# kensho-technologies/pyctcdecode

Measured on AMD Instinct MI355X. Metric: logit-frames/sec (whole node) at beam=100, V=1024, 4-gram LM, higher is better.
Workload: dtype f64

## Files before the change

### pyctcdecode_amd/csrc/frame_prune_hip.hip

```cpp
#include <hip/hip_runtime.h>
#include <hip/hip_fp16.h>
#include <algorithm>
#include <type_traits>
#include <vector>
#include <math.h>
#include <stdlib.h>

#include "backend.h"
#include "set_order.h"
#include "np_f32.h"
#include "set_order_small.h"
#include "np_sum.h"
#include "wave_ops_hip.h"
#include "hip_try.h"
#include "prune_route.h"

namespace ctc {
namespace be {

template <typename T>
__device__ __forceinline__ double ld(const T* p, size_t i) {
  return (double)p[i];
}
struct half_bits { uint16_t u; };
// ... 490 lines not shown
__global__ __launch_bounds__(PRUNE_WAVES * 64) void frame_prune_listed(PruneArgs a, uint32_t cap) {
  extern __shared__ __attribute__((aligned(16))) char smem[];
  const int lane = threadIdx.x & 63;
  const int wave = threadIdx.x >> 6;
  const PruneLds w = prune_lds(smem, wave, (uint32_t)a.max_surv, cap);
  const uint32_t count = a.overflow[3];
  for (uint32_t k = blockIdx.x * PRUNE_WAVES + wave; k < count; k += gridDim.x * PRUNE_WAVES) {
    prune_row_generic<T>(a, a.row_base + (int64_t)a.slow_rows[k], w, lane);
    __builtin_amdgcn_wave_barrier();
    __threadfence_block();
  }
}

__device__ __forceinline__ double exp_nonpos(double d) {
  d = fmax(d, -750.0);
  const double kf = rint(d * 1.44269504088896338700e+00);
  double r = fma(kf, -6.93147180369123816490e-01, d);
  r = fma(kf, -1.90821492927058770002e-10, r);
  double p = 1.6059043836821613e-10;
  p = fma(p, r, 2.08767569878680990e-09);
  p = fma(p, r, 2.50521083854417188e-08);
  p = fma(p, r, 2.75573192239858907e-07);
  p = fma(p, r, 2.75573192239858907e-06);
  p = fma(p, r, 2.48015873015873016e-05);
  p = fma(p, r, 1.98412698412698413e-04);
  p = fma(p, r, 1.38888888888888889e-03);
  p = fma(p, r, 8.33333333333333333e-03);
  p = fma(p, r, 4.16666666666666667e-02);
  p = fma(p, r, 1.66666666666666667e-01);
  p = fma(p, r, 5.00000000000000000e-01);
  p = fma(p, r, 1.0);
  p = fma(p, r, 1.0);
  return ldexp(p, (int)kf);
}

__device__ __forceinline__ double exp_nonpos9(double d) {
  d = fmax(d, -750.0);
  const double kf = rint(d * 1.44269504088896338700e+00);
  double r = fma(kf, -6.93147180369123816490e-01, d);
  r = fma(kf, -1.90821492927058770002e-10, r);
  double p = 2.75573192239858907e-06;
  p = fma(p, r, 2.48015873015873016e-05);
  p = fma(p, r, 1.98412698412698413e-04);
  p = fma(p, r, 1.38888888888888889e-03);
  p = fma(p, r, 8.33333333333333333e-03);
  p = fma(p, r, 4.16666666666666667e-02);
  p = fma(p, r, 1.66666666666666667e-01);
  p = fma(p, r, 5.00000000000000000e-01);
  p = fma(p, r, 1.0);
  p = fma(p, r, 1.0);
  return ldexp(p, (int)kf);
}

typedef float f32x2 __attribute__((ext_vector_type(2)));
__device__ __forceinline__ f32x2 exp_nonpos_f32x2(f32x2 d) {
  d = __builtin_elementwise_max(d, (f32x2)(-80.0f));
  const f32x2 n = __builtin_elementwise_roundeven(d * (f32x2)(1.44269504088896340736f));
  f32x2 r = __builtin_elementwise_fma(n, (f32x2)(-0.693145751953125f), d);
  r = __builtin_elementwise_fma(n, (f32x2)(-1.42860682030941723212e-6f), r);
  f32x2 p = (f32x2)(2.48015873015873016e-05f);
  p = __builtin_elementwise_fma(p, r, (f32x2)(1.98412698412698413e-04f));
  p = __builtin_elementwise_fma(p, r, (f32x2)(1.38888888888888889e-03f));
  p = __builtin_elementwise_fma(p, r, (f32x2)(8.33333333333333333e-03f));
  p = __builtin_elementwise_fma(p, r, (f32x2)(4.16666666666666667e-02f));
  p = __builtin_elementwise_fma(p, r, (f32x2)(1.66666666666666667e-01f));
  p = __builtin_elementwise_fma(p, r, (f32x2)(0.5f));
  p = __builtin_elementwise_fma(p, r, (f32x2)(1.0f));
  p = __builtin_elementwise_fma(p, r, (f32x2)(1.0f));
  f32x2 out;
  out.x = ldexpf(p.x, (int)n.x);
  out.y = ldexpf(p.y, (int)n.y);
  return out;
}

__device__ __forceinline__ double log_ge1(double s) {
  const double y0 = (double)__logf((float)s);
  const double r = fma(s, exp_nonpos(-y0), -1.0);
  return y0 + (r - 0.5 * r * r);
}

template <int NC, bool PK>
__device__ __forceinline__ void prune_row_f32x4(const PruneArgs& a, int64_t row, const PruneLds& w, int lane) {
  const int V = a.n_labels;
  const int u = find_utt(a.utt_row0, a.n_utts, row);
  const bool is_prob = a.pass == 1;
  if (is_prob && a.utt_is_prob[u] != 1u) return;
  const float4* x4 = (const float4*)((const float*)a.utt_logits[u] + (size_t)(row - a.utt_row0[u]) * V);
  const int n4 = V >> 2;
  float4 r[NC];
#pragma unroll
  for (int k = 0; k < NC; ++k) {
    const int i4 = k * 64 + lane;
    r[k] = i4 < n4 ? x4[i4] : make_float4(-INFINITY, -INFINITY, -INFINITY, -INFINITY);
  }
  double mx = 0.0, lse = 0.0;
  const uint32_t ms = (uint32_t)a.max_surv;
  const unsigned long long lt = (1ull << lane) - 1ull;
  if (!is_prob) {
    float mf = -INFINITY;
    float rsf = 0.f;
#pragma unroll
    for (int k = 0; k < NC; ++k) {
      if (k * 64 + lane < n4) {
        mf = fmaxf(fmaxf(mf, fmaxf(r[k].x, r[k].y)), fmaxf(r[k].z, r[k].w));
        rsf += (r[k].x + r[k].y) + (r[k].z + r[k].w);
      }
    }
    double m = wave_max((double)mf);
    double rs = wave_sum((double)rsf);
    if (lane == 0) a.row_sum[row] = rs;
    if (isfinite(m) && rs == rs) {
      const float mfw = (float)m;
      double sl = 0.0;
      float l32 = 0.f;
      const bool np32 = a.f32_np != 0;
      if (np32) l32 = np_log_f32(np_order_exp_sum<float>((const float*)x4, V, mfw, lane, w));
#pragma unroll
      for (int k = 0; k < NC; ++k) {
        if (!np32 && k * 64 + lane < n4) {
          if (PK) {
            const f32x2 e01 = exp_nonpos_f32x2((f32x2){r[k].x - mfw, r[k].y - mfw});
            const f32x2 e23 = exp_nonpos_f32x2((f32x2){r[k].z - mfw, r[k].w - mfw});
            sl += ((double)e01.x + (double)e01.y) + ((double)e23.x + (double)e23.y);
          } else {
            sl += (exp_nonpos9((double)r[k].x - m) + exp_nonpos9((double)r[k].y - m)) +
                  (exp_nonpos9((double)r[k].z - m) + exp_nonpos9((double)r[k].w - m));
          }
        }
      }
      if (!np32) {
        const double s = wave_sum(sl);
        lse = log_ge1(s);
      } else {
        lse = (double)l32;
      }
      int first = 0x7FFFFFFF;
#pragma unroll
      for (int k = NC - 1; k >= 0; --k) {
        const int v0 = (k * 64 + lane) * 4;
        if (k * 64 + lane < n4) {
          first = r[k].w == mfw ? v0 + 3 : first;
          first = r[k].z == mfw ? v0 + 2 : first;
          first = r[k].y == mfw ? v0 + 1 : first;
          first = r[k].x == mfw ? v0 : first;
        }
      }
      first = wave_min_i32(first);
      const double best = np32 ? to_logp_np32(mfw, false, mfw, l32) : to_logp((double)mfw, false, m, lse);
      const double xthr = m + lse + a.token_min_logp;
      const float pre = a.token_min_logp <= -34.538776394910684 ? -INFINITY
                                                                  : __double2float_rd(xthr - (np32 ? 3e-5 * (4.0 + fabs(xthr)) : 1e-6 * (1.0 + fabs(xthr))));
      uint32_t n = 0;
#pragma unroll
      for (int k = 0; k < NC; ++k) {
        const bool in = k * 64 + lane < n4;
        const bool cand = in && (r[k].x >= pre || r[k].y >= pre || r[k].z >= pre || r[k].w >= pre);
        if (__ballot(cand)) {
          const int v0 = (k * 64 + lane) * 4;
          double y0 = -INFINITY, y1 = -INFINITY, y2 = -INFINITY, y3 = -INFINITY;
          if (cand && np32) {
            y0 = to_logp_np32(r[k].x, false, mfw, l32);
            y1 = to_logp_np32(r[k].y, false, mfw, l32);
            y2 = to_logp_np32(r[k].z, false, mfw, l32);
            y3 = to_logp_np32(r[k].w, false, mfw, l32);
          } else if (cand) {
            y0 = to_logp((double)r[k].x, false, m, lse);
            y1 = to_logp((double)r[k].y, false, m, lse);
            y2 = to_logp((double)r[k].z, false, m, lse);
            y3 = to_logp((double)r[k].w, false, m, lse);
          }
          const bool k0 = cand && y0 >= a.token_min_logp, k1 = cand && y1 >= a.token_min_logp;
          const bool k2 = cand && y2 >= a.token_min_logp, k3 = cand && y3 >= a.token_min_logp;
          const unsigned long long b0 = __ballot(k0), b1 = __ballot(k1), b2 = __ballot(k2), b3 = __ballot(k3);
          uint32_t pos = n + (uint32_t)(__popcll(b0 & lt) + __popcll(b1 & lt) + __popcll(b2 & lt) + __popcll(b3 & lt));
          if (k0) { if (pos < ms) { w.asc_id[pos] = (uint16_t)v0; w.asc_lp[pos] = y0; } ++pos; }
          if (k1) { if (pos < ms) { w.asc_id[pos] = (uint16_t)(v0 + 1); w.asc_lp[pos] = y1; } ++pos; }
          if (k2) { if (pos < ms) { w.asc_id[pos] = (uint16_t)(v0 + 2); w.asc_lp[pos] = y2; } ++pos; }
          if (k3) { if (pos < ms) { w.asc_id[pos] = (uint16_t)(v0 + 3); w.asc_lp[pos] = y3; } ++pos; }
          n += (uint32_t)(__popcll(b0) + __popcll(b1) + __popcll(b2) + __popcll(b3));
        }
      }
      prune_finish(a, row, lane, w, n, best, first, true);
      return;
    }
    if (!isfinite(m)) m = 0.0;
    double s = 0.0;
#pragma unroll
    for (int k = 0; k < NC; ++k) {
      if (k * 64 + lane < n4)
        s += (exp((double)r[k].x - m) + exp((double)r[k].y - m)) + (exp((double)r[k].z - m) + exp((double)r[k].w - m));
    }
    s = wave_sum(s);
    mx = m;
    lse = log(s);
  }
  uint32_t n = 0;
  double best = -INFINITY;
  int best_id = 0x7FFFFFFF;
#pragma unroll
  for (int k = 0; k < NC; ++k) {
    const bool in = k * 64 + lane < n4;
    const int v0 = (k * 64 + lane) * 4;
    double y0 = -INFINITY, y1 = -INFINITY, y2 = -INFINITY, y3 = -INFINITY;
    if (in && is_prob && a.f32_np) {
      y0 = to_logp_np32(r[k].x, true, 0.f, 0.f);
      y1 = to_logp_np32(r[k].y, true, 0.f, 0.f);
      y2 = to_logp_np32(r[k].z, true, 0.f, 0.f);
      y3 = to_logp_np32(r[k].w, true, 0.f, 0.f);
    } else if (in) {
      y0 = to_logp((double)r[k].x, is_prob, mx, lse);
      y1 = to_logp((double)r[k].y, is_prob, mx, lse);
      y2 = to_logp((double)r[k].z, is_prob, mx, lse);
      y3 = to_logp((double)r[k].w, is_prob, mx, lse);
    }
    if (in) {
      argmax_take(y0, v0, best, best_id);
      argmax_take(y1, v0 + 1, best, best_id);
      argmax_take(y2, v0 + 2, best, best_id);
      argmax_take(y3, v0 + 3, best, best_id);
    }
    const bool k0 = in && y0 >= a.token_min_logp, k1 = in && y1 >= a.token_min_logp;
    const bool k2 = in && y2 >= a.token_min_logp, k3 = in && y3 >= a.token_min_logp;
    const unsigned long long any = __ballot(k0 || k1 || k2 || k3);
    if (any) {
      const unsigned long long b0 = __ballot(k0), b1 = __ballot(k1), b2 = __ballot(k2), b3 = __ballot(k3);
      uint32_t pos = n + (uint32_t)(__popcll(b0 & lt) + __popcll(b1 & lt) + __popcll(b2 & lt) + __popcll(b3 & lt));
      if (k0) { if (pos < ms) { w.asc_id[pos] = (uint16_t)v0; w.asc_lp[pos] = y0; } ++pos; }
      if (k1) { if (pos < ms) { w.asc_id[pos] = (uint16_t)(v0 + 1); w.asc_lp[pos] = y1; } ++pos; }
      if (k2) { if (pos < ms) { w.asc_id[pos] = (uint16_t)(v0 + 2); w.asc_lp[pos] = y2; } ++pos; }
      if (k3) { if (pos < ms) { w.asc_id[pos] = (uint16_t)(v0 + 3); w.asc_lp[pos] = y3; } ++pos; }
      n += (uint32_t)(__popcll(b0) + __popcll(b1) + __popcll(b2) + __popcll(b3));
    }
  }
  prune_finish(a, row, lane, w, n, best, best_id);
}
template <int NC, bool PK>
__global__ __launch_bounds__(PRUNE_WAVES * 64) void frame_prune_f32x4(PruneArgs a, uint32_t cap) {
  extern __shared__ __attribute__((aligned(16))) char smem[];
  const int lane = threadIdx.x & 63;
  const int wave = threadIdx.x >> 6;
  const int64_t row = a.row_base + (int64_t)blockIdx.x * PRUNE_WAVES + wave;
  if (row >= a.row_base + a.n_rows) return;
  prune_row_f32x4<NC, PK>(a, row, prune_lds(smem, wave, (uint32_t)a.max_surv, cap), lane);
}
template <int NC>
__global__ __launch_bounds__(PRUNE_WAVES * 64) void frame_prune_f32x4_listed(PruneArgs a, uint32_t cap) {
  extern __shared__ __attribute__((aligned(16))) char smem[];
  const int lane = threadIdx.x & 63;
  const int wave = threadIdx.x >> 6;
  const PruneLds w = prune_lds(smem, wave, (uint32_t)a.max_surv, cap);
  const uint32_t count = a.overflow[3];
  for (uint32_t k = blockIdx.x * PRUNE_WAVES + wave; k < count; k += gridDim.x * PRUNE_WAVES) {
    prune_row_f32x4<NC, true>(a, a.row_base + (int64_t)a.slow_rows[k], w, lane);
    __builtin_amdgcn_wave_barrier();
    __threadfence_block();
  }
}

constexpr int PF_ROWS = 64;
constexpr int PF_CAND = 16;
constexpr int PF_WAVES = 3;
constexpr int NP_IL = 2;
constexpr size_t PF_LDS_IDS = (size_t)PF_ROWS * PF_CAND * 2;
constexpr size_t PF_LDS_X = (size_t)PF_ROWS * PF_CAND * 4;
static_assert(PRUNE_FAST_MAX_LABELS - 1 <= (int)SMALL_SET_MAX_ID, "label ids must fit the small set tables");
constexpr size_t PF_LDS = PF_LDS_IDS + PF_LDS_X + (size_t)PF_ROWS * SMALL_SET_SLOTS * 2;

__device__ __forceinline__ f32x2 exp_nonpos_f32x2m(f32x2 d) {
  d.x = fmaxf(d.x, -80.0f);
  d.y = fmaxf(d.y, -80.0f);
  const f32x2 magic = (f32x2)(12582912.0f);
  const f32x2 t = __builtin_elementwise_fma(d, (f32x2)(1.44269504088896340736f), magic);
  const f32x2 n = t - magic;
  f32x2 r = __builtin_elementwise_fma(n, (f32x2)(-0.693145751953125f), d);
  r = __builtin_elementwise_fma(n, (f32x2)(-1.42860682030941723212e-6f), r);
  f32x2 p = (f32x2)(1.98412698412698413e-04f);
  p = __builtin_elementwise_fma(p, r, (f32x2)(1.38888888888888889e-03f));
  p = __builtin_elementwise_fma(p, r, (f32x2)(8.33333333333333333e-03f));
  p = __builtin_elementwise_fma(p, r, (f32x2)(4.16666666666666667e-02f));
  p = __builtin_elementwise_fma(p, r, (f32x2)(1.66666666666666667e-01f));
  p = __builtin_elementwise_fma(p, r, (f32x2)(0.5f));
  p = __builtin_elementwise_fma(p, r, (f32x2)(1.0f));
  p = __builtin_elementwise_fma(p, r, (f32x2)(1.0f));
  f32x2 out;
  out.x = __uint_as_float(__float_as_uint(p.x) + (__float_as_uint(t.x) << 23));
  out.y = __uint_as_float(__float_as_uint(p.y) + (__float_as_uint(t.y) << 23));
  return out;
}

template <int CTRL, int ROW_MASK>
__device__ __forceinline__ float dpp_f32(float ident, float v) {
  return __int_as_float(__builtin_amdgcn_update_dpp(__float_as_int(ident), __float_as_int(v), CTRL, ROW_MASK, 0xf, false));
}
__device__ __forceinline__ float min3_raw(float a, float b, float c) {
  float o;
  asm("v_min3_f32 %0, %1, %2, %3" : "=v"(o) : "v"(a), "v"(b), "v"(c));
  return o;
}
__device__ __forceinline__ float max3_raw(float a, float b, float c) {
  float o;
  asm("v_max3_f32 %0, %1, %2, %3" : "=v"(o) : "v"(a), "v"(b), "v"(c));
  return o;
}
#define CTC_MAX_DPP(V, CTRL) asm volatile("s_nop 1\n\tv_max_f32_dpp %0, %0, %0 " CTRL : "+v"(V))
__device__ __forceinline__ float wave_max_f32(float v) {
  CTC_MAX_DPP(v, "row_shr:1 row_mask:0xf bank_mask:0xf");
  CTC_MAX_DPP(v, "row_shr:2 row_mask:0xf bank_mask:0xf");
  CTC_MAX_DPP(v, "row_shr:4 row_mask:0xf bank_mask:0xf");
  CTC_MAX_DPP(v, "row_shr:8 row_mask:0xf bank_mask:0xf");
  CTC_MAX_DPP(v, "row_bcast:15 row_mask:0xa bank_mask:0xf");
  CTC_MAX_DPP(v, "row_bcast:31 row_mask:0xc bank_mask:0xf");
  asm volatile("s_nop 1" ::: "memory");
  return __int_as_float(__builtin_amdgcn_readlane(__float_as_int(v), 63));
}
__device__ __forceinline__ float wave_sum_f32(float v) {
  v += dpp_f32<0x111, 0xf>(0.f, v);
  v += dpp_f32<0x112, 0xf>(0.f, v);
  v += dpp_f32<0x114, 0xf>(0.f, v);
  v += dpp_f32<0x118, 0xf>(0.f, v);
  v += dpp_f32<0x142, 0xa>(0.f, v);
  v += dpp_f32<0x143, 0xc>(0.f, v);
  return __int_as_float(__builtin_amdgcn_readlane(__float_as_int(v), 63));
}
__device__ __forceinline__ uint32_t lanes_below(uint64_t mask) {
  return __builtin_amdgcn_mbcnt_hi((uint32_t)(mask >> 32), __builtin_amdgcn_mbcnt_lo((uint32_t)mask, 0u));
}

struct LaneTab {
  uint16_t* t;
  __device__ __forceinline__ uint16_t get(uint32_t k) const { return t[k * PF_ROWS]; }
  __device__ __forceinline__ void put(uint32_t k, uint16_t v) { t[k * PF_ROWS] = v; }
};

typedef float PfF4 __attribute__((ext_vector_type(4)));
typedef uint32_t PfU4 __attribute__((ext_vector_type(4)));
template <int DT>
struct PfRaw {
  typedef PfF4 type;
};
template <>
struct PfRaw<2> {
  typedef PfU4 type;
};
template <>
struct PfRaw<3> {
  typedef PfU4 type;
};
template <int DT>
__device__ __forceinline__ float pf_widen(uint32_t h16) {
  return DT == 2 ? __half2float(__ushort_as_half((unsigned short)h16)) : __uint_as_float(h16 << 16);
}

__device__ __forceinline__ f32x2 np_exp_nonpos_pk(f32x2 t) {
#pragma clang fp contract(off)
  f32x2 tc;
  tc.x = fmaxf(t.x, -104.0f);
  tc.y = fmaxf(t.y, -104.0f);
  const f32x2 magic = (f32x2)(12582912.0f);
  f32x2 q = tc * (f32x2)(1.442695040888963407359924681001892137f);
  q = q + magic;
  q = q - magic;
  f32x2 r = __builtin_elementwise_fma(q, (f32x2)(-6.93145752e-1f), tc);
  r = __builtin_elementwise_fma(q, (f32x2)(-1.42860677e-6f), r);
  f32x2 num = __builtin_elementwise_fma((f32x2)(5.082762527590693718096e-04f), r, (f32x2)(6.757896990527504603057e-03f));
  num = __builtin_elementwise_fma(num, r, (f32x2)(5.114512081637298353406e-02f));
  num = __builtin_elementwise_fma(num, r, (f32x2)(2.473615434895520810817e-01f));
  num = __builtin_elementwise_fma(num, r, (f32x2)(7.257664613233124478488e-01f));
  num = __builtin_elementwise_fma(num, r, (f32x2)(9.999999999980870924916e-01f));
  f32x2 den = __builtin_elementwise_fma((f32x2)(2.159509375685829852307e-02f), r, (f32x2)(-2.742335390411667452936e-01f));
  den = __builtin_elementwise_fma(den, r, (f32x2)(1.0f));
  f32x2 p;
#ifdef CTC_NP_SHORT_DIV
  f32x2 y0;
  y0.x = __builtin_amdgcn_rcpf(den.x);
  y0.y = __builtin_amdgcn_rcpf(den.y);
  const f32x2 e = __builtin_elementwise_fma(-den, y0, (f32x2)(1.0f));
  const f32x2 y = __builtin_elementwise_fma(e, y0, y0);
  const f32x2 q0 = num * y;
  const f32x2 rem = __builtin_elementwise_fma(-den, q0, num);
  p = __builtin_elementwise_fma(rem, y, q0);
#else
  p.x = num.x / den.x;
  p.y = num.y / den.y;
#endif
  f32x2 v;
  v.x = ldexpf(p.x, (int)q.x);
  v.y = ldexpf(p.y, (int)q.y);
  v.x = t.x <= -103.97208404541015625f ? 0.0f : v.x;
  v.y = t.y <= -103.97208404541015625f ? 0.0f : v.y;
  return v;
}
template <int N>
__device__ __forceinline__ void np_exp_nonpos_pk_fast_n(const f32x2 (&t)[N], f32x2 (&v)[N]) {
#pragma clang fp contract(off)
  const f32x2 magic = (f32x2)(12582912.0f);
  f32x2 q[N], qm[N], r[N], num[N], den[N], y0[N], q0[N];
#define CTC_STAGE(expr)                      \
  _Pragma("unroll") for (int i = 0; i < N; ++i) { expr; } \
  __builtin_amdgcn_sched_barrier(0);
  CTC_STAGE(q[i] = t[i] * (f32x2)(1.442695040888963407359924681001892137f))
  CTC_STAGE(qm[i] = q[i] + magic)
  CTC_STAGE(q[i] = qm[i] - magic)
  CTC_STAGE(r[i] = __builtin_elementwise_fma(q[i], (f32x2)(-6.93145752e-1f), t[i]))
  CTC_STAGE(r[i] = __builtin_elementwise_fma(q[i], (f32x2)(-1.42860677e-6f), r[i]))
  CTC_STAGE(num[i] = __builtin_elementwise_fma((f32x2)(5.082762527590693718096e-04f), r[i], (f32x2)(6.757896990527504603057e-03f));
            den[i] = __builtin_elementwise_fma((f32x2)(2.159509375685829852307e-02f), r[i], (f32x2)(-2.742335390411667452936e-01f)))
  CTC_STAGE(num[i] = __builtin_elementwise_fma(num[i], r[i], (f32x2)(5.114512081637298353406e-02f));
            den[i] = __builtin_elementwise_fma(den[i], r[i], (f32x2)(1.0f)))
  CTC_STAGE(num[i] = __builtin_elementwise_fma(num[i], r[i], (f32x2)(2.473615434895520810817e-01f));
            y0[i].x = __builtin_amdgcn_rcpf(den[i].x))
  CTC_STAGE(num[i] = __builtin_elementwise_fma(num[i], r[i], (f32x2)(7.257664613233124478488e-01f));
            y0[i].y = __builtin_amdgcn_rcpf(den[i].y))
  CTC_STAGE(num[i] = __builtin_elementwise_fma(num[i], r[i], (f32x2)(9.999999999980870924916e-01f)))
  CTC_STAGE(q0[i] = num[i] * y0[i])
  CTC_STAGE(num[i] = __builtin_elementwise_fma(-den[i], q0[i], num[i]))
  CTC_STAGE(q0[i] = __builtin_elementwise_fma(num[i], y0[i], q0[i]))
  CTC_STAGE(v[i].x = __uint_as_float(__float_as_uint(q0[i].x) + (__float_as_uint(qm[i].x) << 23));
            v[i].y = __uint_as_float(__float_as_uint(q0[i].y) + (__float_as_uint(qm[i].y) << 23)))
#undef CTC_STAGE
}
__device__ __forceinline__ int np_pad(int i) { return i + ((i >> 7) << 3); }
constexpr size_t PF_TABS_BYTES = (size_t)PF_ROWS * SMALL_SET_SLOTS * 2;
__host__ __device__ inline size_t pf_np_rowbuf_bytes(int nc) { return ((size_t)(nc * 256 + nc * 16 + 16) * 4 + 15) & ~(size_t)15; }
__host__ __device__ inline size_t pf_np_extra_lds(int nc, int n_leaf) {
  const size_t ls = (size_t)n_leaf * PF_ROWS * 4;
  return ls + (pf_np_rowbuf_bytes(nc) <= PF_TABS_BYTES ? 0 : pf_np_rowbuf_bytes(nc));
}

template <int NC, int DT, bool AL = true, bool NP = false>
__global__ __launch_bounds__(64) __attribute__((amdgpu_waves_per_eu(NC <= 4 ? PF_WAVES : 1, NC <= 4 ? PF_WAVES : 8))) void frame_prune_fast(PruneArgs a) {
  extern __shared__ __attribute__((aligned(16))) char smem[];
  const int lane = threadIdx.x;
  const int64_t row_lo = a.row_base + (int64_t)blockIdx.x * PF_ROWS;
  const int64_t row_end = a.row_base + a.n_rows;
  if (row_lo >= row_end) return;
  const int nrows = (int)(row_end - row_lo < (int64_t)PF_ROWS ? row_end - row_lo : (int64_t)PF_ROWS);
  uint16_t* ar_id = (uint16_t*)smem;
  float* ar_x = (float*)(smem + PF_LDS_IDS);
  uint16_t* tabs = (uint16_t*)(smem + PF_LDS_IDS + PF_LDS_X);
  static_assert(!NP || DT == 0, "numpy-order sums: float32 rows");
  float* np_ls = (float*)(smem + PF_LDS);
  float* np_rb = pf_np_rowbuf_bytes(NC) <= PF_TABS_BYTES ? (float*)tabs : (float*)(smem + PF_LDS + (a.np_uniform8 ? 0 : (size_t)a.np_n_leaf * PF_ROWS * 4));
  constexpr bool WIDE = DT == 0;
  constexpr int NL = WIDE ? NC : NC / 2;
  constexpr int PER = WIDE ? 4 : 8;
  static_assert(WIDE || NC % 2 == 0, "16-bit rows: two float4 groups per load");
  static_assert(AL || WIDE, "element-wise loads: float32 rows only");
  typedef typename PfRaw<DT>::type Raw;
  const int V = a.n_labels;
  const int n4 = AL ? V / PER : (V + 3) / 4;
  const float tminf = (float)a.token_min_logp;
  auto id_of = [&](int k, int e) { return WIDE ? (k * 64 + lane) * 4 + e : ((k >> 1) * 64 + lane) * 8 + (k & 1) * 4 + e; };
  auto in_row = [&](int k) { return (WIDE ? k : (k >> 1)) * 64 + lane < n4; };

  typedef const int64_t __attribute__((address_space(4))) * ConstI64;
  typedef const void* const __attribute__((address_space(4))) * ConstPtrs;
  typedef const Raw __attribute__((address_space(1))) * GlobalRaw;
  const ConstI64 row0_c = (ConstI64)a.utt_row0;
  const ConstPtrs logits_c = (ConstPtrs)a.utt_logits;
  int u = __builtin_amdgcn_readfirstlane(find_utt(a.utt_row0, a.n_utts, row_lo));
  int64_t u_r0 = row0_c[u], u_r1 = row0_c[u + 1];
  const char __attribute__((address_space(1))) * u_base = (const char __attribute__((address_space(1)))*)logits_c[u];
  auto load_row = [&](int64_t row, Raw(&r)[NL]) {
    while (row >= u_r1) {
      ++u;
      u_r0 = u_r1;
      u_r1 = row0_c[u + 1];
      u_base = (const char __attribute__((address_space(1)))*)logits_c[u];
    }
    const GlobalRaw x4 = (GlobalRaw)(u_base + (size_t)(row - u_r0) * V * (WIDE ? 4 : 2));
#pragma unroll
    for (int k = 0; k < NL; ++k) {
      const int i4 = k * 64 + lane;
      if constexpr (!AL) {
        const float __attribute__((address_space(1)))* xf = (const float __attribute__((address_space(1)))*)x4;
        const int e0 = i4 * 4;
        Raw v;
        v.x = xf[e0 < V ? e0 : 0];
        v.y = xf[e0 + 1 < V ? e0 + 1 : 0];
        v.z = xf[e0 + 2 < V ? e0 + 2 : 0];
        v.w = xf[e0 + 3 < V ? e0 + 3 : 0];
        r[k] = v;
      } else {
        r[k] = x4[i4 < n4 ? i4 : 0];
      }
    }
  };
  auto widen = [&](const Raw(&raw)[NL], float4(&r)[NC]) {
    const float ninf = -INFINITY;
    if constexpr (WIDE) {
#pragma unroll
      for (int k = 0; k < NC; ++k) {
        r[k] = make_float4(raw[k].x, raw[k].y, raw[k].z, raw[k].w);
        if constexpr (!AL) {
          const int e0 = (k * 64 + lane) * 4;
          if (e0 >= V) r[k].x = ninf;
          if (e0 + 1 >= V) r[k].y = ninf;
          if (e0 + 2 >= V) r[k].z = ninf;
          if (e0 + 3 >= V) r[k].w = ninf;
        } else if (!in_row(k)) {
          r[k] = make_float4(ninf, ninf, ninf, ninf);
        }
      }
    } else {
#pragma unroll
      for (int k = 0; k < NL; ++k) {
        r[2 * k] = make_float4(pf_widen<DT>(raw[k].x & 0xFFFFu), pf_widen<DT>(raw[k].x >> 16), pf_widen<DT>(raw[k].y & 0xFFFFu),
                               pf_widen<DT>(raw[k].y >> 16));
        r[2 * k + 1] = make_float4(pf_widen<DT>(raw[k].z & 0xFFFFu), pf_widen<DT>(raw[k].z >> 16), pf_widen<DT>(raw[k].w & 0xFFFFu),
                                   pf_widen<DT>(raw[k].w >> 16));
        if (!in_row(2 * k)) {
          r[2 * k] = make_float4(ninf, ninf, ninf, ninf);
          r[2 * k + 1] = make_float4(ninf, ninf, ninf, ninf);
        }
      }
    }
  };

  float my_m = 0.f, my_rs = 0.f, my_s32 = 1.0f;
  double my_s = 1.0;
  int my_first = 0;
  uint32_t my_cnt = 0;

  int np_off0 = 0, np_len0 = 0;
  if constexpr (NP) {
    const int leaf = lane >> 3;
    if (leaf < a.np_n_leaf) {
      np_off0 = a.np_leaf[2 * leaf];
      np_len0 = a.np_leaf[2 * leaf + 1];
    }
  }
  auto np_accumulate = [&](int i) {
    __builtin_amdgcn_fence(__ATOMIC_SEQ_CST, "wavefront");
    __builtin_amdgcn_wave_barrier();
    const int g = lane >> 3, j = lane & 7;
    const int nl = a.np_n_leaf;
    for (int base = 0; base < nl; base += 8) {
      const int leaf = base + g;
      const bool mine = leaf < nl;
      int off = np_off0, len = np_len0;
      if (base > 0) {
        off = len = 0;
        if (mine) {
          off = a.np_leaf[2 * leaf];
          len = a.np_leaf[2 * leaf + 1];
        }
      }
      float res = 0.f;
      if (len == 128 && (off & 127) == 0) {
        const float* q = np_rb + np_pad(off) + j;
        float t0 = q[0], t1 = q[8], t2 = q[16], t3 = q[24], t4 = q[32], t5 = q[40], t6 = q[48], t7 = q[56];
        float t8 = q[64], t9 = q[72], t10 = q[80], t11 = q[88], t12 = q[96], t13 = q[104], t14 = q[112], t15 = q[120];
        float rr = t0 + t1;
        rr = rr + t2; rr = rr + t3; rr = rr + t4; rr = rr + t5; rr = rr + t6; rr = rr + t7; rr = rr + t8;
        rr = rr + t9; rr = rr + t10; rr = rr + t11; rr = rr + t12; rr = rr + t13; rr = rr + t14; rr = rr + t15;
        res = rr;
      } else if (len >= 8) {
        const int body = len - (len & 7);
        float rr = np_rb[np_pad(off + j)];
        for (int t = 8; t < body; t += 8) rr = rr + np_rb[np_pad(off + t + j)];
        res = rr;
      }
      res = res + dpp_f32<0xB1, 0xf>(0.f, res);
      res = res + dpp_f32<0x4E, 0xf>(0.f, res);
      res = res + dpp_f32<0x141, 0xf>(0.f, res);
      if ((len & 7) != 0 || len < 8) {
        const int body = len >= 8 ? len - (len & 7) : 0;
        if (len < 8) res = 0.f;
        for (int t = body; t < len; ++t) res = res + np_rb[np_pad(off + t)];
      }
      if (a.np_uniform8) {
        float t = res + dpp_f32<0x128, 0xf>(0.f, res);
        t = t + dpp_f32<0x142, 0xa>(0.f, t);
        t = t + dpp_f32<0x143, 0xc>(0.f, t);
        const float total = __int_as_float(__builtin_amdgcn_readlane(__float_as_int(t), 63));
        if (lane == i) my_s32 = total;
      } else if (mine && j == 0) {
        np_ls[leaf * PF_ROWS + i] = res;
      }
    }
    __builtin_amdgcn_fence(__ATOMIC_SEQ_CST, "wavefront");
    __builtin_amdgcn_wave_barrier();
  };

  auto phase_a = [&](int i, const Raw(&raw)[NL]) -> uint32_t {
    float4 r[NC];
    widen(raw, r);
    float mf = -INFINITY, rsf;
#pragma unroll
    for (int k = 0; k < NC; ++k) mf = max3_raw(max3_raw(mf, r[k].x, r[k].y), r[k].z, r[k].w);
    if (!AL) {
      rsf = 0.f;
#pragma unroll
      for (int k = 0; k < NC; ++k) {
        const int e0 = (k * 64 + lane) * 4;
        rsf += ((e0 < V ? r[k].x : 0.f) + (e0 + 1 < V ? r[k].y : 0.f)) + ((e0 + 2 < V ? r[k].z : 0.f) + (e0 + 3 < V ? r[k].w : 0.f));
      }
    } else if (n4 == NL * 64) {
      f32x2 rs2 = (f32x2)(0.f);
#pragma unroll
      for (int k = 0; k < NC; ++k) rs2 += (f32x2){r[k].x, r[k].y} + (f32x2){r[k].z, r[k].w};
      rsf = rs2.x + rs2.y;
    } else {
      rsf = 0.f;
#pragma unroll
      for (int k = 0; k < NC; ++k) rsf += in_row(k) ? (r[k].x + r[k].y) + (r[k].z + r[k].w) : 0.f;
    }
    const float m = wave_max_f32(mf);
    const float rs = wave_sum_f32(rsf);
    uint32_t cnt = 0xFFFFu;
    int first = 0;
    double s = 1.0;
    bool clean = isfinite(m) && rs == rs;
    if constexpr (NP) {
      float lo = INFINITY;
#pragma unroll
      for (int k = 0; k < NC; ++k) {
        if constexpr (AL) {
          if (n4 == NL * 64 || in_row(k)) lo = min3_raw(min3_raw(lo, r[k].x, r[k].y), r[k].z, r[k].w);
        } else {
          const int e0 = (k * 64 + lane) * 4;
          lo = fminf(lo, fminf(fminf(e0 < V ? r[k].x : lo, e0 + 1 < V ? r[k].y : lo), fminf(e0 + 2 < V ? r[k].z : lo, e0 + 3 < V ? r[k].w : lo)));
        }
      }
      if (clean && __ballot(!(lo - m > -87.0f)) != 0ull) clean = false;
    }
    if (clean) {
      if constexpr (NP) {
        f32x2 approx = (f32x2)(0.f);
        const f32x2 mm2 = (f32x2)(m);
        constexpr int IL = NC % NP_IL == 0 ? NP_IL : 1;
        f32x2 ex[NC][2];
#pragma unroll
        for (int k0 = 0; k0 < NC; k0 += IL) {
          f32x2 tin[2 * IL], tout[2 * IL];
#pragma unroll
          for (int j = 0; j < IL; ++j) {
            tin[2 * j] = (f32x2){r[k0 + j].x, r[k0 + j].y} - mm2;
            tin[2 * j + 1] = (f32x2){r[k0 + j].z, r[k0 + j].w} - mm2;
          }
          np_exp_nonpos_pk_fast_n<2 * IL>(tin, tout);
#pragma unroll
          for (int j = 0; j < IL; ++j) {
            ex[k0 + j][0] = tout[2 * j];
            ex[k0 + j][1] = tout[2 * j + 1];
          }
        }
#pragma unroll
        for (int k = 0; k < NC; ++k) {
          const f32x2 e01 = ex[k][0], e23 = ex[k][1];
          bool inside = true;
          if constexpr (AL) inside = n4 == NL * 64 || in_row(k);
          else inside = (k * 64 + lane) * 4 + 3 < V;
          if (inside) approx += e01 + e23;
          *(float4*)(np_rb + np_pad((k * 64 + lane) * 4)) = make_float4(e01.x, e01.y, e23.x, e23.y);
        }
        s = (double)wave_sum_f32(approx.x + approx.y);
      } else {
      f32x2 acc = (f32x2)(0.f);
      const f32x2 mm = (f32x2)(m);
#pragma unroll
      for (int k = 0; k < NC; ++k) {
        acc += exp_nonpos_f32x2m((f32x2){r[k].x, r[k].y} - mm);
        acc += exp_nonpos_f32x2m((f32x2){r[k].z, r[k].w} - mm);
      }
      s = wave_sum((double)(acc.x + acc.y));
      }
      const float xthr = (m + __logf((float)s)) + tminf;
      const float pre = xthr - 3e-5f * (4.0f + fabsf(xthr));
      cnt = 0;
#pragma unroll
      for (int k = 0; k < NC; ++k) {
#pragma unroll
        for (int e = 0; e < 4; ++e) {
          const float x = e == 0 ? r[k].x : e == 1 ? r[k].y : e == 2 ? r[k].z : r[k].w;
          const bool c = x >= pre;
          const uint64_t mk = __ballot(c);
          if (mk) {
            const uint32_t pos = cnt + lanes_below(mk);
            if (c && pos < (uint32_t)PF_CAND) {
              ar_id[pos * PF_ROWS + i] = (uint16_t)id_of(k, e);
              ar_x[pos * PF_ROWS + i] = x;
            }
            cnt += (uint32_t)__popcll(mk);
          }
        }
      }
      if (cnt == 0) {
        first = 0x7FFFFFFF;
#pragma unroll
        for (int k = 0; k < NC; ++k) {
          if (first == 0x7FFFFFFF || (!WIDE && (k & 1))) {
            const uint64_t b0 = __ballot(r[k].x == m), b1 = __ballot(r[k].y == m), b2 = __ballot(r[k].z == m),
                           b3 = __ballot(r[k].w == m);
            const uint64_t any = b0 | b1 | b2 | b3;
            if (any) {
              const int l = __builtin_ctzll(any);
              const int e = ((b0 >> l) & 1ull) ? 0 : ((b1 >> l) & 1ull) ? 1 : ((b2 >> l) & 1ull) ? 2 : 3;
              const int cand = WIDE ? (k * 64 + l) * 4 + e : ((k >> 1) * 64 + l) * 8 + (k & 1) * 4 + e;
              if (cand < first) first = cand;
            }
          }
        }
      }
      if constexpr (NP) np_accumulate(i);
    }
    if (lane == i) {
      my_m = m;
      my_rs = rs;
      my_s = s;
      my_first = first;
      my_cnt = cnt;
    }
    return cnt;
  };

  const int64_t row_last = row_lo + nrows - 1;
  auto row_at = [&](int i) { return row_lo + i < row_last ? row_lo + i : row_last; };
  if constexpr (NC <= 4) {
    Raw ra[NL], rb[NL], rc[NL];
    load_row(row_at(0), ra);
    load_row(row_at(1), rb);
    for (int i = 0; i < nrows; i += 3) {
      load_row(row_at(i + 2), rc);
      phase_a(i, ra);
      load_row(row_at(i + 3), ra);
      if (i + 1 < nrows) phase_a(i + 1, rb);
      load_row(row_at(i + 4), rb);
      if (i + 2 < nrows) phase_a(i + 2, rc);
    }
  } else if constexpr (NC <= 8) {
    Raw ra[NL], rb[NL];
    load_row(row_at(0), ra);
    for (int i = 0; i < nrows; i += 2) {
      load_row(row_at(i + 1), rb);
      phase_a(i, ra);
      load_row(row_at(i + 2), ra);
      if (i + 1 < nrows) phase_a(i + 1, rb);
    }
  } else {
    Raw ra[NL];
    for (int i = 0; i < nrows; ++i) {
      load_row(row_at(i), ra);
      phase_a(i, ra);
    }
  }
  __syncthreads();

  const int64_t row = row_lo + lane;
  const uint32_t ms = (uint32_t)a.max_surv;
  bool slow = false;
  if (lane < nrows) {
    const uint32_t cnt = my_cnt;
    slow = cnt > (uint32_t)PF_CAND;
    if (!slow) {
      const double s = my_s;
      const double md = (double)my_m;
      double lse = 0.0;
      float l32 = 0.f;
      if constexpr (NP) {
        float s32 = my_s32;
        if (!a.np_uniform8) {
          for (int q = 0; q + 1 < a.np_n_leaf; ++q) {
            const int dst = a.np_prog[2 * q], src = a.np_prog[2 * q + 1];
            np_ls[dst * PF_ROWS + lane] = np_ls[dst * PF_ROWS + lane] + np_ls[src * PF_ROWS + lane];
          }
          s32 = np_ls[lane];
        }
        l32 = np_log_f32(s32);
      } else {
        lse = log_ge1(s);
      }
      auto logp_of = [&](float x) { return NP ? to_logp_np32(x, false, my_m, l32) : to_logp((double)x, false, md, lse); };
      const double best = logp_of(my_m);
      uint16_t* ids = ar_id + lane;
      float* xs = ar_x + lane;
      uint32_t n = 0;
      uint32_t first = cnt > 0 ? 0xFFFFu : (uint32_t)my_first;
      for (uint32_t j = 0; j < cnt; ++j) {
        const uint16_t id = ids[j * PF_ROWS];
        const float x = xs[j * PF_ROWS];
        if (x == my_m && id < first) first = id;
        if (logp_of(x) >= a.token_min_logp) {
          uint32_t p = n;
          while (p > 0 && ids[(p - 1) * PF_ROWS] > id) {
            ids[p * PF_ROWS] = ids[(p - 1) * PF_ROWS];
            xs[p * PF_ROWS] = xs[(p - 1) * PF_ROWS];
            --p;
          }
          ids[p * PF_ROWS] = id;
          xs[p * PF_ROWS] = x;
          ++n;
        }
      }
      slow = n > SMALL_SET_MAX_KEYS || n >= ms;
      if (!slow) {
        LaneTab tab{tabs + lane};
        const SmallSet r = small_set_order(tab, n, [ids](uint32_t k) { return (uint32_t)ids[k * PF_ROWS]; },
                                           first);
        uint16_t* out_id = a.surv_id + (size_t)row * ms;
        double* out_lp = a.surv_lp + (size_t)row * ms;
        uint32_t pos = 0;
        for (uint32_t k = 0; k <= r.mask; ++k) {
          const uint16_t v = tab.get(r.base + k);
          if (v != SMALL_SET_EMPTY) {
            const uint32_t pay = v >> SMALL_SET_ID_BITS;
            out_id[pos] = (uint16_t)(v & SMALL_SET_ID_MASK);
            out_lp[pos] = pay == SMALL_SET_ARGMAX ? best : logp_of(xs[pay * PF_ROWS]);
            ++pos;
          }
        }
        a.surv_cnt[row] = pos;
        a.row_sum[row] = (double)my_rs;
      }
    }
  }
  const uint64_t sm = __ballot(slow);
  if (sm) {
    uint32_t base = 0;
    if (lane == 0) base = atomicAdd(&a.overflow[3], (uint32_t)__popcll(sm));
    base = (uint32_t)__builtin_amdgcn_readfirstlane((int)base);
    if (slow) a.slow_rows[base + lanes_below(sm)] = (uint32_t)(row - a.row_base);
  }
}

struct NpPlan {
  int V = -1, n_leaf = 0, uniform8 = 0;
  uint16_t* d_leaf = nullptr;
  uint8_t* d_prog = nullptr;
};
static int np_plan_node(int off, int n, std::vector<uint16_t>& leaf, std::vector<uint8_t>& prog) {
  if (n <= 128) {
    leaf.push_back((uint16_t)off);
    leaf.push_back((uint16_t)n);
    return (int)leaf.size() / 2 - 1;
  }
  int n2 = n / 2;
  n2 -= n2 % 8;
  const int l = np_plan_node(off, n2, leaf, prog), r = np_plan_node(off + n2, n - n2, leaf, prog);
  prog.push_back((uint8_t)l);
  prog.push_back((uint8_t)r);
  return l;
}
static int np_plan_for(int V, hipStream_t stream, NpPlan** out, std::string* err) {
  static NpPlan plans[4];
  static int next = 0;
  for (NpPlan& p : plans)
    if (p.V == V) {
      *out = &p;
      return 0;
    }
  NpPlan& p = plans[next];
  next = (next + 1) % 4;
  std::vector<uint16_t> leaf;
  std::vector<uint8_t> prog;
  np_plan_node(0, V, leaf, prog);
  prog.push_back(0);
  prog.push_back(0);
  HIP_TRY(hipStreamSynchronize(stream));
  if (p.d_leaf) (void)hipFree(p.d_leaf);
  if (p.d_prog) (void)hipFree(p.d_prog);
  p.d_leaf = nullptr;
  p.d_prog = nullptr;
  p.V = -1;
  HIP_TRY(hipMalloc((void**)&p.d_leaf, leaf.size() * 2));
  HIP_TRY(hipMalloc((void**)&p.d_prog, prog.size()));
  HIP_TRY(hipMemcpy(p.d_leaf, leaf.data(), leaf.size() * 2, hipMemcpyHostToDevice));
  HIP_TRY(hipMemcpy(p.d_prog, prog.data(), prog.size(), hipMemcpyHostToDevice));
  p.n_leaf = (int)leaf.size() / 2;
  p.uniform8 = (p.n_leaf == 1 || p.n_leaf == 2 || p.n_leaf == 4 || p.n_leaf == 8) ? 1 : 0;
  for (size_t k = 0; k < leaf.size(); k += 2)
    if (leaf[k + 1] != 128 || (leaf[k] & 127) != 0) p.uniform8 = 0;
  p.V = V;
  *out = &p;
  return 0;
}

template <class F>
static int with_nc(int nc, F f) {
  switch (nc) {
    case 1: return f(std::integral_constant<int, 1>());
    case 2: return f(std::integral_constant<int, 2>());
    case 3: return f(std::integral_constant<int, 3>());
    case 4: return f(std::integral_constant<int, 4>());
    case 5: return f(std::integral_constant<int, 5>());
    case 6: return f(std::integral_constant<int, 6>());
    case 7: return f(std::integral_constant<int, 7>());
    case 8: return f(std::integral_constant<int, 8>());
    case 12: return f(std::integral_constant<int, 12>());
    default: return f(std::integral_constant<int, 16>());
  }
}
template <class F>
static int with_flag(bool b, F f) { return b ? f(std::true_type()) : f(std::false_type()); }
template <class K, class... Args>
static int launch_lds(K kern, dim3 grid, dim3 block, size_t lds, hipStream_t stream, std::string* err, const Args&... args) {
  HIP_TRY(hipFuncSetAttribute((const void*)kern, hipFuncAttributeMaxDynamicSharedMemorySize, (int)lds));
  hipLaunchKernelGGL(kern, grid, block, lds, stream, args...);
  return 0;
}

int launch_prune_on(const PruneArgs& a_in, hipStream_t stream, std::string* err) {
  PruneArgs a = a_in;
  const PruneRoute rt = prune_route(PruneShape{a.dtype, a.n_labels, a.rows_aligned4 != 0, a.rows_aligned16 != 0, a.pass,
                                               a.slow_rows != nullptr, a.n_rows, a.dense_hint != 0,
                                               prune_exp_of(getenv("CTCDEC_PRUNE_EXP")),
                                               prune_per_row_forced(getenv("CTCDEC_PRUNE_KERNEL"))});
  a.f32_np = rt.np ? 1 : 0;
  a.np_prog = nullptr;
  a.np_leaf = nullptr;
  a.np_n_leaf = 0;
  a.np_uniform8 = 0;
  if (a.n_rows > 0) {
    const uint32_t cap = set_table_cap((uint32_t)a.max_surv + 1);
    const size_t lds = prune_lds_bytes((size_t)a.max_surv, cap) * PRUNE_WAVES;
    if (lds > 160 * 1024) {
      if (err) *err = "token_min_logp admits too many labels per frame for the LDS set tables";
      return -1;
    }
    const dim3 grid((unsigned)((a.n_rows + PRUNE_WAVES - 1) / PRUNE_WAVES)), block(PRUNE_WAVES * 64);
    const dim3 fgrid((unsigned)((a.n_rows + PF_ROWS - 1) / PF_ROWS)), fblock(64);
    const dim3 rest((unsigned)std::min<int64_t>((a.n_rows + PRUNE_WAVES - 1) / PRUNE_WAVES, 2048));
    int rc = 0;
    switch (rt.kernel) {
      case PRUNE_FAST_F32: {
        size_t flds = PF_LDS;
        if (rt.np) {
          NpPlan* plan = nullptr;
          if (np_plan_for(a.n_labels, stream, &plan, err)) return -1;
          a.np_leaf = plan->d_leaf;
          a.np_prog = plan->d_prog;
          a.np_n_leaf = plan->n_leaf;
          a.np_uniform8 = plan->uniform8;
          flds += pf_np_extra_lds(rt.nc, plan->uniform8 ? 0 : plan->n_leaf);
        }
        rc = with_nc(rt.nc, [&](auto nc) { return with_flag(rt.al, [&](auto al) { return with_flag(rt.np, [&](auto np) {
          constexpr int NC = decltype(nc)::value;
          return launch_lds(frame_prune_fast<NC, 0, decltype(al)::value, decltype(np)::value>, fgrid, fblock, flds, stream, err, a);
        }); }); });
        if (rc) return rc;
        if (rt.listed == PRUNE_LISTED_F32X4) rc = with_nc(rt.nc, [&](auto nc) {
          constexpr int NC = decltype(nc)::value <= 4 ? decltype(nc)::value : 4;
          return launch_lds(frame_prune_f32x4_listed<NC>, rest, block, lds, stream, err, a, cap);
        });
        else rc = launch_lds(frame_prune_listed<float>, rest, block, lds, stream, err, a, cap);
        break;
      }
      case PRUNE_FAST_16:
        rc = with_flag(a.dtype == 2, [&](auto f16) { return with_flag(rt.nc == 2, [&](auto one_load) {
          constexpr int NC = decltype(one_load)::value ? 2 : 4, DT = decltype(f16)::value ? 2 : 3;
          hipLaunchKernelGGL((frame_prune_fast<NC, DT>), fgrid, fblock, PF_LDS, stream, a);
          return launch_lds(frame_prune_listed<std::conditional_t<DT == 2, half_bits, bf16_bits>>, rest, block, lds, stream, err, a, cap);
        }); });
        break;
      case PRUNE_ROW_F32X4:
        rc = with_nc(rt.nc, [&](auto nc) { return with_flag(rt.pk, [&](auto pk) {
          constexpr int NC = decltype(nc)::value <= 4 ? decltype(nc)::value : 4;
          return launch_lds(frame_prune_f32x4<NC, decltype(pk)::value>, grid, block, lds, stream, err, a, cap);
        }); });
        break;
      case PRUNE_ROW_GENERIC:
        if (a.dtype == 0) rc = launch_lds(frame_prune<float>, grid, block, lds, stream, err, a, cap);
        else if (a.dtype == 1) rc = launch_lds(frame_prune<double>, grid, block, lds, stream, err, a, cap);
        else if (a.dtype == 2) rc = launch_lds(frame_prune<half_bits>, grid, block, lds, stream, err, a, cap);
        else rc = launch_lds(frame_prune<bf16_bits>, grid, block, lds, stream, err, a, cap);
        break;
    }
    if (rc) return rc;
    HIP_TRY(hipGetLastError());
  }
  if (a.n_utts > 0) {
    if (a.pass == 0) hipLaunchKernelGGL(utt_sniff, dim3((unsigned)a.n_utts), dim3(64), 0, stream, a);
    else hipLaunchKernelGGL(utt_recount, dim3((unsigned)a.n_utts), dim3(64), 0, stream, a);
    HIP_TRY(hipGetLastError());
  }
  return 0;
}

int launch_sniff_exact_on(const PruneArgs& a, hipStream_t stream, std::string* err) {
  if (a.n_utts > 0) {
    hipLaunchKernelGGL(utt_sniff_exact, dim3((unsigned)a.n_utts), dim3(256), 0, stream, a);
    HIP_TRY(hipGetLastError());
  }
  return 0;
}

}
}
```

Measured before the change: 191.5 million.

## Specialize frame-prune phase for full rows and streamline row addressing

Adds a compile-time FULL-row specialization so aligned rows that fill every lane skip per-lane in-row masking in widen, min, and sum loops. It also fuses the wave max and sum DPP reductions into one interleaved asm block, and replaces per-row 64-bit utterance offset math with a precomputed row pointer plus 32-bit relative index. A dedicated uniform-8 numpy-order accumulator is split out, and a cheaper log2-based log is used. Duplicating the row loop per specialization grows code size and may change register pressure.

Result: faster. 198.2 million, median of 6 (+3.5%).

```diff
diff --git a/pyctcdecode_amd/csrc/frame_prune_hip.hip b/pyctcdecode_amd/csrc/frame_prune_hip.hip
--- a/pyctcdecode_amd/csrc/frame_prune_hip.hip
+++ b/pyctcdecode_amd/csrc/frame_prune_hip.hip
@@ -816,17 +816,20 @@
   asm("v_max3_f32 %0, %1, %2, %3" : "=v"(o) : "v"(a), "v"(b), "v"(c));
   return o;
 }
-#define CTC_MAX_DPP(V, CTRL) asm volatile("s_nop 1\n\tv_max_f32_dpp %0, %0, %0 " CTRL : "+v"(V))
-__device__ __forceinline__ float wave_max_f32(float v) {
-  CTC_MAX_DPP(v, "row_shr:1 row_mask:0xf bank_mask:0xf");
-  CTC_MAX_DPP(v, "row_shr:2 row_mask:0xf bank_mask:0xf");
-  CTC_MAX_DPP(v, "row_shr:4 row_mask:0xf bank_mask:0xf");
-  CTC_MAX_DPP(v, "row_shr:8 row_mask:0xf bank_mask:0xf");
-  CTC_MAX_DPP(v, "row_bcast:15 row_mask:0xa bank_mask:0xf");
-  CTC_MAX_DPP(v, "row_bcast:31 row_mask:0xc bank_mask:0xf");
-  asm volatile("s_nop 1" ::: "memory");
-  return __int_as_float(__builtin_amdgcn_readlane(__float_as_int(v), 63));
-}
+#define CTC_MAX_SUM_DPP(CTRL) "v_max_f32_dpp %0, %0, %0 " CTRL "\n\tv_add_f32_dpp %1, %1, %1 " CTRL "\n\ts_nop 0\n\t"
+__device__ __forceinline__ void wave_max_sum_f32(float& mx, float& sm) {
+  asm volatile("s_nop 1\n\t"
+               CTC_MAX_SUM_DPP("row_shr:1 row_mask:0xf bank_mask:0xf")
+               CTC_MAX_SUM_DPP("row_shr:2 row_mask:0xf bank_mask:0xf")
+               CTC_MAX_SUM_DPP("row_shr:4 row_mask:0xf bank_mask:0xf")
+               CTC_MAX_SUM_DPP("row_shr:8 row_mask:0xf bank_mask:0xf")
+               CTC_MAX_SUM_DPP("row_bcast:15 row_mask:0xa bank_mask:0xf")
+               CTC_MAX_SUM_DPP("row_bcast:31 row_mask:0xc bank_mask:0xf")
+               : "+v"(mx), "+v"(sm));
+  mx = __int_as_float(__builtin_amdgcn_readlane(__float_as_int(mx), 63));
+  sm = __int_as_float(__builtin_amdgcn_readlane(__float_as_int(sm), 63));
+}
+#undef CTC_MAX_SUM_DPP
 __device__ __forceinline__ float wave_sum_f32(float v) {
   v += dpp_f32<0x111, 0xf>(0.f, v);
   v += dpp_f32<0x112, 0xf>(0.f, v);
@@ -948,7 +951,7 @@
   const int64_t row_lo = a.row_base + (int64_t)blockIdx.x * PF_ROWS;
   const int64_t row_end = a.row_base + a.n_rows;
   if (row_lo >= row_end) return;
-  const int nrows = (int)(row_end - row_lo < (int64_t)PF_ROWS ? row_end - row_lo : (int64_t)PF_ROWS);
+  const int nrows = __builtin_amdgcn_readfirstlane((int)(row_end - row_lo < (int64_t)PF_ROWS ? row_end - row_lo : (int64_t)PF_ROWS));
   uint16_t* ar_id = (uint16_t*)smem;
   float* ar_x = (float*)(smem + PF_LDS_IDS);
   uint16_t* tabs = (uint16_t*)(smem + PF_LDS_IDS + PF_LDS_X);
@@ -963,6 +966,7 @@
   typedef typename PfRaw<DT>::type Raw;
   const int V = a.n_labels;
   const int n4 = AL ? V / PER : (V + 3) / 4;
+  const bool full_row = AL && n4 == NL * 64;
   const float tminf = (float)a.token_min_logp;
   auto id_of = [&](int k, int e) { return WIDE ? (k * 64 + lane) * 4 + e : ((k >> 1) * 64 + lane) * 8 + (k & 1) * 4 + e; };
   auto in_row = [&](int k) { return (WIDE ? k : (k >> 1)) * 64 + lane < n4; };
@@ -972,17 +976,22 @@
   typedef const Raw __attribute__((address_space(1))) * GlobalRaw;
   const ConstI64 row0_c = (ConstI64)a.utt_row0;
   const ConstPtrs logits_c = (ConstPtrs)a.utt_logits;
+  const uint32_t row_bytes = (uint32_t)V * (WIDE ? 4u : 2u);
+  auto rel_end = [&](int64_t r1) {
+    return __builtin_amdgcn_readfirstlane((int)(r1 - row_lo < (int64_t)PF_ROWS ? r1 - row_lo : (int64_t)PF_ROWS));
+  };
   int u = __builtin_amdgcn_readfirstlane(find_utt(a.utt_row0, a.n_utts, row_lo));
-  int64_t u_r0 = row0_c[u], u_r1 = row0_c[u + 1];
-  const char __attribute__((address_space(1))) * u_base = (const char __attribute__((address_space(1)))*)logits_c[u];
-  auto load_row = [&](int64_t row, Raw(&r)[NL]) {
-    while (row >= u_r1) {
+  int64_t u_r1 = row0_c[u + 1];
+  int u_end = rel_end(u_r1);
+  uint64_t u_row = (uint64_t)logits_c[u] + (uint64_t)(row_lo - row0_c[u]) * row_bytes;
+  auto load_row = [&](int i, Raw(&r)[NL]) __attribute__((always_inline)) {
+    while (i >= u_end) {
       ++u;
-      u_r0 = u_r1;
+      u_row = (uint64_t)logits_c[u] + (uint64_t)(row_lo - u_r1) * row_bytes;
       u_r1 = row0_c[u + 1];
-      u_base = (const char __attribute__((address_space(1)))*)logits_c[u];
-    }
-    const GlobalRaw x4 = (GlobalRaw)(u_base + (size_t)(row - u_r0) * V * (WIDE ? 4 : 2));
+      u_end = rel_end(u_r1);
+    }
+    const GlobalRaw x4 = (GlobalRaw)(u_row + (uint64_t)((uint32_t)i * row_bytes));
 #pragma unroll
     for (int k = 0; k < NL; ++k) {
       const int i4 = k * 64 + lane;
@@ -1000,7 +1009,8 @@
       }
     }
   };
-  auto widen = [&](const Raw(&raw)[NL], float4(&r)[NC]) {
+  auto widen = [&](auto full_c, const Raw(&raw)[NL], float4(&r)[NC]) __attribute__((always_inline)) {
+    constexpr bool FULL = decltype(full_c)::value;
     const float ninf = -INFINITY;
     if constexpr (WIDE) {
 #pragma unroll
@@ -1012,8 +1022,6 @@
           if (e0 + 1 >= V) r[k].y = ninf;
           if (e0 + 2 >= V) r[k].z = ninf;
           if (e0 + 3 >= V) r[k].w = ninf;
-        } else if (!in_row(k)) {
-          r[k] = make_float4(ninf, ninf, ninf, ninf);
         }
       }
     } else {
@@ -1023,11 +1031,12 @@
                                pf_widen<DT>(raw[k].y >> 16));
         r[2 * k + 1] = make_float4(pf_widen<DT>(raw[k].z & 0xFFFFu), pf_widen<DT>(raw[k].z >> 16), pf_widen<DT>(raw[k].w & 0xFFFFu),
                                    pf_widen<DT>(raw[k].w >> 16));
-        if (!in_row(2 * k)) {
-          r[2 * k] = make_float4(ninf, ninf, ninf, ninf);
-          r[2 * k + 1] = make_float4(ninf, ninf, ninf, ninf);
-        }
-      }
+      }
+    }
+    if constexpr (AL && !FULL) {
+#pragma unroll
+      for (int k = 0; k < NC; ++k)
+        if (!in_row(k)) r[k] = make_float4(ninf, ninf, ninf, ninf);
     }
   };
 
@@ -1044,7 +1053,7 @@
       np_len0 = a.np_leaf[2 * leaf + 1];
     }
   }
-  auto np_accumulate = [&](int i) {
+  auto np_accumulate = [&](int i) __attribute__((always_inline)) {
     __builtin_amdgcn_fence(__ATOMIC_SEQ_CST, "wavefront");
     __builtin_amdgcn_wave_barrier();
     const int g = lane >> 3, j = lane & 7;
@@ -1083,23 +1092,39 @@
         if (len < 8) res = 0.f;
         for (int t = body; t < len; ++t) res = res + np_rb[np_pad(off + t)];
       }
-      if (a.np_uniform8) {
-        float t = res + dpp_f32<0x128, 0xf>(0.f, res);
-        t = t + dpp_f32<0x142, 0xa>(0.f, t);
-        t = t + dpp_f32<0x143, 0xc>(0.f, t);
-        const float total = __int_as_float(__builtin_amdgcn_readlane(__float_as_int(t), 63));
-        if (lane == i) my_s32 = total;
-      } else if (mine && j == 0) {
-        np_ls[leaf * PF_ROWS + i] = res;
-      }
+      if (mine && j == 0) np_ls[leaf * PF_ROWS + i] = res;
     }
     __builtin_amdgcn_fence(__ATOMIC_SEQ_CST, "wavefront");
     __builtin_amdgcn_wave_barrier();
   };
-
-  auto phase_a = [&](int i, const Raw(&raw)[NL]) -> uint32_t {
+  const float* np_q8 = np_rb + np_pad(np_off0) + (lane & 7);
+  auto np_accumulate8 = [&](int i) __attribute__((always_inline)) {
+    __builtin_amdgcn_fence(__ATOMIC_SEQ_CST, "wavefront");
+    __builtin_amdgcn_wave_barrier();
+    const float* q = np_q8;
+    float t0 = q[0], t1 = q[8], t2 = q[16], t3 = q[24], t4 = q[32], t5 = q[40], t6 = q[48], t7 = q[56];
+    float t8 = q[64], t9 = q[72], t10 = q[80], t11 = q[88], t12 = q[96], t13 = q[104], t14 = q[112], t15 = q[120];
+    float rr = t0 + t1;
+    rr = rr + t2; rr = rr + t3; rr = rr + t4; rr = rr + t5; rr = rr + t6; rr = rr + t7; rr = rr + t8;
+    rr = rr + t9; rr = rr + t10; rr = rr + t11; rr = rr + t12; rr = rr + t13; rr = rr + t14; rr = rr + t15;
+    float res = rr;
+    res = res + dpp_f32<0xB1, 0xf>(0.f, res);
+    res = res + dpp_f32<0x4E, 0xf>(0.f, res);
+    res = res + dpp_f32<0x141, 0xf>(0.f, res);
+    if (a.np_n_leaf < 8) res = np_len0 != 0 ? res : 0.f;
+    float t = res + dpp_f32<0x128, 0xf>(0.f, res);
+    t = t + dpp_f32<0x142, 0xa>(0.f, t);
+    t = t + dpp_f32<0x143, 0xc>(0.f, t);
+    const float total = __int_as_float(__builtin_amdgcn_readlane(__float_as_int(t), 63));
+    if (lane == i) my_s32 = total;
+    __builtin_amdgcn_fence(__ATOMIC_SEQ_CST, "wavefront");
+    __builtin_amdgcn_wave_barrier();
+  };
+
+  auto phase_a = [&](auto full_c, int i, const Raw(&raw)[NL]) __attribute__((always_inline)) -> uint32_t {
+    constexpr bool FULL = decltype(full_c)::value;
     float4 r[NC];
-    widen(raw, r);
+    widen(full_c, raw, r);
     float mf = -INFINITY, rsf;
 #pragma unroll
     for (int k = 0; k < NC; ++k) mf = max3_raw(max3_raw(mf, r[k].x, r[k].y), r[k].z, r[k].w);
@@ -1110,7 +1135,7 @@
         const int e0 = (k * 64 + lane) * 4;
         rsf += ((e0 < V ? r[k].x : 0.f) + (e0 + 1 < V ? r[k].y : 0.f)) + ((e0 + 2 < V ? r[k].z : 0.f) + (e0 + 3 < V ? r[k].w : 0.f));
       }
-    } else if (n4 == NL * 64) {
+    } else if (FULL) {
       f32x2 rs2 = (f32x2)(0.f);
 #pragma unroll
       for (int k = 0; k < NC; ++k) rs2 += (f32x2){r[k].x, r[k].y} + (f32x2){r[k].z, r[k].w};
@@ -1120,21 +1145,26 @@
 #pragma unroll
       for (int k = 0; k < NC; ++k) rsf += in_row(k) ? (r[k].x + r[k].y) + (r[k].z + r[k].w) : 0.f;
     }
-    const float m = wave_max_f32(mf);
-    const float rs = wave_sum_f32(rsf);
+    wave_max_sum_f32(mf, rsf);
+    const float m = mf, rs = rsf;
     uint32_t cnt = 0xFFFFu;
     int first = 0;
     double s = 1.0;
     bool clean = isfinite(m) && rs == rs;
     if constexpr (NP) {
       float lo = INFINITY;
-#pragma unroll
-      for (int k = 0; k < NC; ++k) {
-        if constexpr (AL) {
-          if (n4 == NL * 64 || in_row(k)) lo = min3_raw(min3_raw(lo, r[k].x, r[k].y), r[k].z, r[k].w);
-        } else {
-          const int e0 = (k * 64 + lane) * 4;
-          lo = fminf(lo, fminf(fminf(e0 < V ? r[k].x : lo, e0 + 1 < V ? r[k].y : lo), fminf(e0 + 2 < V ? r[k].z : lo, e0 + 3 < V ? r[k].w : lo)));
+      if constexpr (FULL) {
+#pragma unroll
+        for (int k = 0; k < NC; ++k) lo = min3_raw(min3_raw(lo, r[k].x, r[k].y), r[k].z, r[k].w);
+      } else {
+#pragma unroll
+        for (int k = 0; k < NC; ++k) {
+          if constexpr (AL) {
+            if (in_row(k)) lo = min3_raw(min3_raw(lo, r[k].x, r[k].y), r[k].z, r[k].w);
+          } else {
+            const int e0 = (k * 64 + lane) * 4;
+            lo = fminf(lo, fminf(fminf(e0 < V ? r[k].x : lo, e0 + 1 < V ? r[k].y : lo), fminf(e0 + 2 < V ? r[k].z : lo, e0 + 3 < V ? r[k].w : lo)));
+          }
         }
       }
       if (clean && __ballot(!(lo - m > -87.0f)) != 0ull) clean = false;
@@ -1161,13 +1191,19 @@
           }
         }
 #pragma unroll
-        for (int k = 0; k < NC; ++k) {
-          const f32x2 e01 = ex[k][0], e23 = ex[k][1];
-          bool inside = true;
-          if constexpr (AL) inside = n4 == NL * 64 || in_row(k);
-          else inside = (k * 64 + lane) * 4 + 3 < V;
-          if (inside) approx += e01 + e23;
-          *(float4*)(np_rb + np_pad((k * 64 + lane) * 4)) = make_float4(e01.x, e01.y, e23.x, e23.y);
+        for (int k = 0; k < NC; ++k)
+          *(float4*)(np_rb + np_pad((k * 64 + lane) * 4)) = make_float4(ex[k][0].x, ex[k][0].y, ex[k][1].x, ex[k][1].y);
+        if constexpr (FULL) {
+#pragma unroll
+          for (int k = 0; k < NC; ++k) approx += ex[k][0] + ex[k][1];
+        } else {
+#pragma unroll
+          for (int k = 0; k < NC; ++k) {
+            bool inside;
+            if constexpr (AL) inside = in_row(k);
+            else inside = (k * 64 + lane) * 4 + 3 < V;
+            if (inside) approx += ex[k][0] + ex[k][1];
+          }
         }
         s = (double)wave_sum_f32(approx.x + approx.y);
       } else {
@@ -1180,7 +1216,7 @@
       }
       s = wave_sum((double)(acc.x + acc.y));
       }
-      const float xthr = (m + __logf((float)s)) + tminf;
+      const float xthr = (m + __builtin_amdgcn_logf((float)s) * 0.693147180559945309f) + tminf;
       const float pre = xthr - 3e-5f * (4.0f + fabsf(xthr));
       cnt = 0;
 #pragma unroll
@@ -1217,47 +1253,57 @@
           }
         }
       }
-      if constexpr (NP) np_accumulate(i);
+      if constexpr (NP) {
+        if (a.np_uniform8) np_accumulate8(i);
+        else np_accumulate(i);
+      }
     }
     if (lane == i) {
       my_m = m;
       my_rs = rs;
-      my_s = s;
+      if constexpr (!NP) my_s = s;
       my_first = first;
       my_cnt = cnt;
     }
     return cnt;
   };
 
-  const int64_t row_last = row_lo + nrows - 1;
-  auto row_at = [&](int i) { return row_lo + i < row_last ? row_lo + i : row_last; };
-  if constexpr (NC <= 4) {
-    Raw ra[NL], rb[NL], rc[NL];
-    load_row(row_at(0), ra);
-    load_row(row_at(1), rb);
-    for (int i = 0; i < nrows; i += 3) {
-      load_row(row_at(i + 2), rc);
-      phase_a(i, ra);
-      load_row(row_at(i + 3), ra);
-      if (i + 1 < nrows) phase_a(i + 1, rb);
-      load_row(row_at(i + 4), rb);
-      if (i + 2 < nrows) phase_a(i + 2, rc);
-    }
-  } else if constexpr (NC <= 8) {
-    Raw ra[NL], rb[NL];
-    load_row(row_at(0), ra);
-    for (int i = 0; i < nrows; i += 2) {
-      load_row(row_at(i + 1), rb);
-      phase_a(i, ra);
-      load_row(row_at(i + 2), ra);
-      if (i + 1 < nrows) phase_a(i + 1, rb);
-    }
+  auto row_at = [&](int i) { return i < nrows - 1 ? i : nrows - 1; };
+  auto rows = [&](auto full_c) __attribute__((always_inline)) {
+    if constexpr (NC <= 4) {
+      Raw ra[NL], rb[NL], rc[NL];
+      load_row(row_at(0), ra);
+      load_row(row_at(1), rb);
+      for (int i = 0; i < nrows; i += 3) {
+        load_row(row_at(i + 2), rc);
+        phase_a(full_c, i, ra);
+        load_row(row_at(i + 3), ra);
+        if (i + 1 < nrows) phase_a(full_c, i + 1, rb);
+        load_row(row_at(i + 4), rb);
+        if (i + 2 < nrows) phase_a(full_c, i + 2, rc);
+      }
+    } else if constexpr (NC <= 8) {
+      Raw ra[NL], rb[NL];
+      load_row(row_at(0), ra);
+      for (int i = 0; i < nrows; i += 2) {
+        load_row(row_at(i + 1), rb);
+        phase_a(full_c, i, ra);
+        load_row(row_at(i + 2), ra);
+        if (i + 1 < nrows) phase_a(full_c, i + 1, rb);
+      }
+    } else {
+      Raw ra[NL];
+      for (int i = 0; i < nrows; ++i) {
+        load_row(row_at(i), ra);
+        phase_a(full_c, i, ra);
+      }
+    }
+  };
+  if constexpr (AL) {
+    if (full_row) rows(std::true_type());
+    else rows(std::false_type());
   } else {
-    Raw ra[NL];
-    for (int i = 0; i < nrows; ++i) {
-      load_row(row_at(i), ra);
-      phase_a(i, ra);
-    }
+    rows(std::false_type());
   }
   __syncthreads();
 
```
